# CZY-Code/PHNet

Hardware: AMD Instinct MI355X
Metric: clips/s (5x3x320x800) fwd+bwd (higher is better)
Workload: dtype f32 storage / accumulation, every product as an EXACT three-term bf16 split (6 bf16 MFMAs, f32-MFMA accuracy); 1 GPU; 5-frame clip 3x320x800, resnet34 + router + lane head, fwd+bwd+AdamW, 1 clip/GPU/step, random-init weights; parallelism=dp1, launch=hipGraph replay of the whole step

## Files before the change

### include/phnet_hip.h

```cpp
#ifndef PHNET_HIP_H
#define PHNET_HIP_H
#include <stdint.h>
#ifdef __cplusplus
extern "C" {
#endif

#define PHNET_OK 0
#define PHNET_ERR_ARG (-1)
#define PHNET_ERR_WORKSPACE (-2)
#define PHNET_ERR_LAUNCH (-3)
#define PHNET_ABI_VERSION 1

int phnet_abi_version(void);

int phnet_lane_nms(const float* rows, const float* scores, const int32_t* counts, int64_t frames,
                   int64_t k_max, int32_t n_offsets, float thresh, int64_t top_k,
                   int64_t* keep, int64_t* num_to_keep, int64_t* parent, void* stream);

int phnet_lane_decode(const float* lines, int64_t frames, int32_t N, int32_t n_offsets, float conf_thresh,
                      float nms_thresh, int64_t top_k, float img_w, uint8_t* keep_mask, int64_t* num,
                      int64_t* keep_c, int64_t* anchors, int64_t* anchors_sorted, float* kept_rows, void* stream);

int phnet_lane_points(const float* kept_rows, const int64_t* num, const float* prior_ys, int64_t F, int32_t L, int32_t S,
                      float* points, int32_t* count, int32_t* lanes_num, int32_t* slot, void* stream);
// ... 14 lines not shown
int phnet_lane_targets_aug(const float* points, const int32_t* counts, const int32_t* lanes_num, const double* offsets_ys, float* out,
                           int64_t F, int32_t Lin, int32_t P, int32_t R, int32_t S, double img_h, double img_w, double strip_size,
                           double crop, double src_w, double scale_x, double scale_y, int32_t flip, const int32_t* flip2,
                           const double* fwd, void* stream);
int phnet_lane_targets_clip(const float* points, const int32_t* counts, const int32_t* lanes_num, const double* offsets_ys, float* out,
                            int64_t F, int32_t Lin, int32_t P, int32_t R, int32_t S, double img_h, double img_w, double strip_size,
                            double crop, double src_w, double scale_x, double scale_y, int32_t flip, const int32_t* flip2,
                            const double* fwd, int32_t clip, int32_t* frag_count, void* stream);

int phnet_roi_pool_fwd(const float* fmap, const float* xs, const float* ys, float* out, float* out_cp,
                       int32_t B, int32_t N, int32_t P, int32_t h, int32_t w, int32_t C, void* stream);
int phnet_roi_pool_bwd(const float* dout, const float* fmap, const float* xs, const float* ys,
                       float* dmap, float* dxs,
                       int32_t B, int32_t N, int32_t P, int32_t h, int32_t w, int32_t C, void* stream);

int phnet_conv2d_fwd(const float* x, const float* w, const float* bias, float* y,
                     int32_t N, int32_t Hi, int32_t Wi, int32_t Ci, int32_t Co, int32_t R, int32_t S,
                     int32_t stride, int32_t pad, int32_t relu, void* workspace, uint64_t ws_bytes, void* stream);
uint64_t phnet_conv2d_stats_blocks(int64_t M, int32_t Co, int32_t K, uint64_t ws_bytes);
int phnet_conv2d_fwd_fused(const float* x, const float* w, const float* bias, const float* addend, float* y, float* stats,
                           int32_t N, int32_t Hi, int32_t Wi, int32_t Ci, int32_t Co, int32_t R, int32_t S,
                           int32_t stride, int32_t pad, int32_t relu, void* workspace, uint64_t ws_bytes, void* stream);
int phnet_conv2d_dgrad(const float* dy, const float* w, const float* addend, float* dx,
                       int32_t N, int32_t Hi, int32_t Wi, int32_t Ci, int32_t Co, int32_t R, int32_t S,
                       int32_t stride, int32_t pad, void* workspace, uint64_t ws_bytes, void* stream);
int phnet_conv3p_applies(int64_t M, int32_t Ca, int32_t Nn);
uint64_t phnet_conv3p_packed_bytes(int32_t Co, int32_t Ci);
int phnet_conv3p_pack(const float* w, void* packed, int32_t Co, int32_t Ci, int32_t dgrad, void* stream);
int phnet_conv3p_pack_jobs(const void* jobs, int32_t njobs, int64_t total, void* stream);
uint64_t phnet_conv3p_stats_blocks(int64_t M, int32_t Ca, int32_t Nn, uint64_t ws_bytes);
int phnet_conv3p_fwd(const float* x, const void* packed, const float* bias, const float* addend, float* y, float* stats,
                     int32_t N, int32_t H, int32_t W, int32_t Ca, int32_t Nn, int32_t relu,
                     void* workspace, uint64_t ws_bytes, void* stream);
int phnet_conv2d_plan(int64_t M, int32_t Co, int32_t K, uint64_t ws_bytes, int32_t* bm, int32_t* bn, int32_t* splits,
                      int32_t* k_tile);
int phnet_conv2d_kernel(int32_t dgrad, int32_t N, int32_t Hi, int32_t Wi, int32_t Ci, int32_t Co, int32_t R, int32_t S,
                        int32_t stride, int32_t pad, uint64_t ws_bytes, char* name, int32_t name_cap, int32_t* splits);
int phnet_conv2d_wgrad_kernel(int32_t N, int32_t Hi, int32_t Wi, int32_t Ci, int32_t Co, int32_t R, int32_t S, int32_t stride,
                              int32_t pad, int32_t has_dbias, uint64_t ws_bytes, char* name, int32_t name_cap, int32_t* splits);
int phnet_linear_bwd_kernel(int32_t M, int32_t K, int32_t N, int32_t has_relu_mask, char* name, int32_t name_cap);
int phnet_conv3p_kernel(int64_t M, int32_t Ca, int32_t Nn, uint64_t ws_bytes, char* name, int32_t name_cap, int32_t* splits);
uint64_t phnet_conv2d_wgrad_workspace(int32_t N, int32_t Hi, int32_t Wi, int32_t Ci, int32_t Co,
                                      int32_t R, int32_t S, int32_t stride, int32_t pad);
int phnet_conv2d_wgrad(const float* dy, const float* x, float* dw, float* dbias,
                       int32_t N, int32_t Hi, int32_t Wi, int32_t Ci, int32_t Co, int32_t R, int32_t S,
                       int32_t stride, int32_t pad, int32_t accumulate, void* workspace, uint64_t ws_bytes, void* stream);
int phnet_linear_bwd_fusable(int64_t M, int64_t K, int64_t N);
int phnet_linear_bwd(const float* dy, const float* x, const float* w, const float* relu_y, float* dx, float* dw, float* dbias,
                     int32_t M, int32_t K, int32_t N, int32_t accumulate, void* stream);
int phnet_nchw3_to_nhwc4(const float* x, float* y, int32_t N, int32_t H, int32_t W, void* stream);
int phnet_pad_channels(const float* src, float* dst, int64_t rows, int32_t cs, int32_t cd, void* stream);

uint64_t phnet_ipc_buffer_bytes(int32_t world, uint64_t max_bytes);
int phnet_ipc_alloc(uint64_t bytes, void** ptr);
int phnet_ipc_free(void* ptr);
int phnet_ipc_get_handle(void* ptr, void* handle64);
int phnet_ipc_open_handle(const void* handle64, void** ptr);
int phnet_ipc_close_handle(void* ptr);
int phnet_oneshot_allreduce(void* data, int32_t count, int32_t dtype, const void* peers, int32_t rank, int32_t world,
                            int32_t cap, void* ctrl, void* stream);

uint64_t phnet_channel_partials_size(int64_t M, int32_t C);
int phnet_bn_fwd_stats(const float* x, int64_t M, int32_t C, float eps, float momentum,
                       const float* gamma, const float* beta, float* running_mean, float* running_var,
                       float* save_mean, float* save_invstd, float* scale, float* shift,
                       float* partial, int32_t training, void* stream);
int phnet_bn_finalize_partials(const float* partial, int64_t nblk, int64_t M, int32_t C, float eps, float momentum,
                               const float* gamma, const float* beta, float* running_mean, float* running_var,
                               float* save_mean, float* save_invstd, float* scale, float* shift, void* stream);
int phnet_bn_apply(const float* x, const float* scale, const float* shift, const float* residual, float* y,
                   int64_t M, int32_t C, int32_t relu, void* stream);
int phnet_bn_bwd(const float* dy, const float* x, const float* y, const float* save_mean,
                 const float* save_invstd, const float* gamma, float* dx, float* dres,
                 float* dgamma, float* dbeta, float* partial, float* c1, float* c2,
                 int64_t M, int32_t C, int32_t relu, int32_t dres_accumulate, int32_t param_accumulate, void* stream);

int phnet_bn_bwd_reduce(const float* dy, const float* x, const float* y, const float* mean, const float* invstd,
                        float* sums, float* partial, float* c1_scratch, float* c2_scratch,
                        int64_t M, int32_t C, int32_t relu, void* stream);
int phnet_bn_bwd_apply(const float* dy, const float* x, const float* y, const float* mean, const float* invstd,
                       const float* gamma, const float* c1, const float* c2, float* dx, float* dres,
                       int64_t M, int32_t C, int32_t relu, int32_t dres_accumulate, void* stream);

int phnet_bn_local_sums(const float* x, int64_t M, int32_t C, float* partial, double* sums, void* stream);
int phnet_bn_partials_to_sums(const float* partial, int64_t nblk, int64_t M, int32_t C, double* sums, void* stream);
int phnet_bn_finalize_sums(const double* sums, int32_t C, float eps, float momentum, const float* gamma, const float* beta,
                           float* running_mean, float* running_var, float* save_mean, float* save_invstd,
                           float* scale, float* shift, void* stream);
int phnet_bn_bwd_apply_sums(const float* dy, const float* x, const float* y, const float* mean, const float* invstd,
                            const float* gamma, const float* sums, const double* count, float* c1, float* c2,
                            float* dx, float* dres, int64_t M, int32_t C, int32_t relu, int32_t dres_accumulate, void* stream);

int phnet_preprocess_u8(const uint8_t* frames, float* out, uint8_t* out_u8,
                        const int32_t* xi, const int16_t* xc, const int32_t* yi, const int16_t* yc,
                        int32_t T, int32_t H0, int32_t W0, int32_t crop_top, int32_t out_h, int32_t out_w, int32_t flip,
                        int32_t layout, const float* mean3_host, const float* std3_host, void* stream);
int phnet_preprocess_yuv(const uint8_t* frames, float* out, uint8_t* out_u8,
                         const int32_t* xi, const int16_t* xc, const int32_t* yi, const int16_t* yc,
                         int32_t T, int32_t H0, int32_t W0, int32_t crop_top, int32_t out_h, int32_t out_w, int32_t flip, int32_t layout,
                         int32_t format, int64_t frame_stride, int32_t pitch, int64_t chroma_offset,
                         const int32_t* csc_host, const float* mean3_host, const float* std3_host, void* stream);

int phnet_augment_u8(const uint8_t* frames, float* out, uint8_t* out_u8, const int32_t* flip2, const double* inv, const int32_t* table,
                     int32_t T, int32_t H, int32_t W, int32_t layout, const float* mean3_host, const float* std3_host, void* stream);

int phnet_augment_stencil_u8(const uint8_t* frames, float* out, uint8_t* out_u8, const int32_t* flip2, const double* inv,
                             const int32_t* table, const int32_t* stencil, uint8_t* staged, int32_t T, int32_t H, int32_t W, int32_t layout,
                             const float* mean3_host, const float* std3_host, void* stream);
// ... 197 lines not shown
```

### include/phnet_hip_tuning.h

```cpp
#ifndef PHNET_HIP_TUNING_H
#define PHNET_HIP_TUNING_H
#include <stdint.h>
#ifdef __cplusplus
extern "C" {
#endif

int phnet_tune_force_conv_tile(int32_t bm, int32_t bn, int32_t splits);
int phnet_tune_force_k_tile(int32_t k_tile);
int phnet_tune_wgrad(int32_t allow_bm128, int32_t target_blocks);
int phnet_tune_mma(int32_t mode);
int phnet_conv3p_tune(int32_t target_workgroups);
int phnet_tune_gate_wave(int32_t on);
int phnet_tune_dyn_mfma(int32_t on);
int phnet_tune_reset(void);
int phnet_tune_mma_get(void);

#ifdef __cplusplus
}
#endif
#endif
```

### phnet_amd/csrc/conv3p.hip

```cpp
#include <cstdio>
#include "igemm.h"
#include "tuning.h"

using namespace igemm;

namespace {

struct P3Shape {
    int N, H, W;
    int Ca, Nn;
    int splits, units_per_split;
};

constexpr int P3_BM = 128, P3_ROWS = P3_BM + 2, P3_THREADS = 256;
constexpr int P3_APITCH = 48;
constexpr int P3_ZROW = P3_ROWS;
constexpr int P3_APLANE = (P3_ROWS + 1) * P3_APITCH, P3_AIMG = 3 * P3_APLANE;
constexpr int P3_PFB = 3;
constexpr size_t P3_LDS = 2 * P3_AIMG + 3 * 512;

struct P3PackJob { const float* w; unsigned char* dst; int Co, Ci, dgrad, pad_; long first; };

__device__ __forceinline__ void conv3p_pack_item(const float* __restrict__ w, unsigned char* __restrict__ packed, int Co, int Ci,
                                                 int dgrad, long i)
// ... 331 lines not shown
{
    if (!w || !packed || Co < 16 || Ci < 16) return PHNET_ERR_ARG;
    const int Ca = dgrad ? Co : Ci, Nn = dgrad ? Ci : Co;
    if ((Ca % 16) || (Nn % 32)) return PHNET_ERR_ARG;
    const long total = (long)9 * (Ca / 16) * (Nn / 32) * 64;
    hipLaunchKernelGGL(conv3p_pack_kernel, dim3((unsigned)cdiv(total, 256)), dim3(256), 0, (hipStream_t)stream,
                       w, (unsigned char*)packed, Co, Ci, dgrad);
    return phnet_launch_status();
}

PHNET_API int phnet_conv3p_pack_jobs(const void* jobs, int32_t njobs, int64_t total, void* stream)
{
    if (!jobs || njobs < 1 || total < 1) return PHNET_ERR_ARG;
    hipLaunchKernelGGL(conv3p_pack_jobs_kernel, dim3((unsigned)cdiv((long)total, 256)), dim3(256), 0, (hipStream_t)stream,
                       (const P3PackJob*)jobs, njobs, (long)total);
    return phnet_launch_status();
}

PHNET_API uint64_t phnet_conv3p_stats_blocks(int64_t M, int32_t Ca, int32_t Nn, uint64_t ws_bytes)
{
    if (!p3_applies((long)M, Ca, Nn)) return 0;
    const P3Plan p = p3_plan((long)M, Ca, Nn, (size_t)ws_bytes);
    return (uint64_t)(p.splits > 1 ? cdiv((long)M * Nn / 4, 256 * P3_RCH) : cdiv((long)M, P3_BM) * (P3_BM / 64));
}

PHNET_API int phnet_conv3p_kernel(int64_t M, int32_t Ca, int32_t Nn, uint64_t ws_bytes, char* name, int32_t name_cap, int32_t* splits)
{
    if (!p3_applies((long)M, Ca, Nn) || !name || name_cap < 1 || !splits) return PHNET_ERR_ARG;
    const P3Plan p = p3_plan((long)M, Ca, Nn, (size_t)ws_bytes);
    *splits = p.splits;
    return p3_kernel_name(p, name, name_cap);
}

PHNET_API int phnet_conv3p_fwd(const float* x, const void* packed, const float* bias, const float* addend, float* y, float* stats,
                               int32_t N, int32_t H, int32_t W, int32_t Ca, int32_t Nn, int32_t relu,
                               void* workspace, uint64_t ws_bytes, void* stream)
{
    if (N < 0 || H < 1 || W < 2 || Ca < 16 || Nn < 64) return PHNET_ERR_ARG;
    if (N == 0) return PHNET_OK;
    const long M = (long)N * H * W;
    if (!x || !packed || !y || !p3_applies(M, Ca, Nn)) return PHNET_ERR_ARG;
    if (stats && (bias || addend || relu || (Nn & (Nn - 1)) || Nn > 1024)) return PHNET_ERR_ARG;
    const P3Plan p = p3_plan(M, Ca, Nn, workspace ? (size_t)ws_bytes : 0);
    P3Shape g{N, H, W, Ca, Nn, p.splits, p.units_per_split};
    float* dst = p.splits > 1 ? (float*)workspace : y;
    hipStream_t st = (hipStream_t)stream;
    if (p.fn == 2)
        hipLaunchKernelGGL(conv3p_kernel<2>, dim3((unsigned)p.tiles, 1, (unsigned)p.splits), dim3(P3_THREADS), P3_LDS, st,
                           x, (const unsigned char*)packed, bias, addend, dst, g, relu, p.splits > 1 ? (float*)nullptr : stats);
    else
        hipLaunchKernelGGL(conv3p_kernel<1>, dim3((unsigned)p.tiles, 1, (unsigned)p.splits), dim3(P3_THREADS), P3_LDS, st,
                           x, (const unsigned char*)packed, bias, addend, dst, g, relu, p.splits > 1 ? (float*)nullptr : stats);
    if (p.splits > 1) {
        const long total4 = M * Nn / 4;
        hipLaunchKernelGGL(conv3p_reduce_kernel, dim3((unsigned)cdiv(total4, stats ? 256 * P3_RCH : 256)), dim3(256), 0, st,
                           (const float*)workspace, y, bias, addend, total4, Nn, p.splits, relu, stats);
    }
    return phnet_launch_status();
}
```

### phnet_amd/csrc/norm.hip

```cpp
#include "common.h"

namespace {

typedef float f32x4 __attribute__((ext_vector_type(4)));
constexpr int NT = 256;

template <int MODE>
__global__ __launch_bounds__(NT) void channel_partials_kernel(
    const float* __restrict__ x, const float* __restrict__ dy, const float* __restrict__ y,
    const float* __restrict__ mean, const float* __restrict__ invstd,
    float* __restrict__ partial, long M, int C, long rows_per_block, int relu)
{
    extern __shared__ f32x4 red[];
    const int lanes_per_row = C >> 2;
    const int rows_at_once = NT / lanes_per_row;
    const int cl = threadIdx.x % lanes_per_row, rl = threadIdx.x / lanes_per_row;
    const long r0 = (long)blockIdx.x * rows_per_block;
    const long r1 = min(M, r0 + rows_per_block);
    f32x4 s0 = {0.f, 0.f, 0.f, 0.f}, s1 = {0.f, 0.f, 0.f, 0.f};
    f32x4 mu = {0.f, 0.f, 0.f, 0.f}, is = {0.f, 0.f, 0.f, 0.f};
    if (MODE == 1) {
        mu = *reinterpret_cast<const f32x4*>(mean + cl * 4);
        is = *reinterpret_cast<const f32x4*>(invstd + cl * 4);
    }
    for (long r = r0 + rl; r < r1; r += rows_at_once) {
        const size_t o = (size_t)r * C + cl * 4;
        const f32x4 xv = *reinterpret_cast<const f32x4*>(x + o);
        if (MODE == 0) {
            s0 += xv;
            s1 += xv * xv;
        } else {
            f32x4 g = *reinterpret_cast<const f32x4*>(dy + o);
            if (relu) {
                const f32x4 yv = *reinterpret_cast<const f32x4*>(y + o);
                g.x = yv.x > 0.f ? g.x : 0.f; g.y = yv.y > 0.f ? g.y : 0.f;
                g.z = yv.z > 0.f ? g.z : 0.f; g.w = yv.w > 0.f ? g.w : 0.f;
            }
            s0 += g;
            s1 += g * ((xv - mu) * is);
        }
    }
    red[threadIdx.x] = s0;
    red[NT + threadIdx.x] = s1;
    __syncthreads();
    if (rl == 0) {
        for (int k = 1; k < rows_at_once; ++k) {
            s0 += red[k * lanes_per_row + cl];
            s1 += red[NT + k * lanes_per_row + cl];
        }
        float* p = partial + (size_t)blockIdx.x * 2 * C;
        *reinterpret_cast<f32x4*>(p + cl * 4) = s0;
        *reinterpret_cast<f32x4*>(p + C + cl * 4) = s1;
    }
}

__device__ __forceinline__ double wave_sum_f64(double v) {
#pragma unroll
    for (int off = 32; off > 0; off >>= 1) v += __shfl_xor(v, off, 64);
    return v;
}

constexpr int FIN_CH = 8, FIN_NT = 1024, FIN_G = FIN_NT / FIN_CH;

__device__ __forceinline__ void finalize_column_sums(const float* __restrict__ partial, int nblk, int C, double* red, double& s0, double& s1)
{
    const int cl = threadIdx.x % FIN_CH, g = threadIdx.x / FIN_CH;
    const int c = blockIdx.x * FIN_CH + cl;
    double a = 0.0, b = 0.0;
    if (c < C) {
        constexpr int U = 8;
        for (int r = g; r < nblk; r += U * FIN_G) {
            float v[U], w[U];
#pragma unroll
            for (int u = 0; u < U; ++u) {
                const int rr = r + u * FIN_G;
                const size_t o = (size_t)(rr < nblk ? rr : g) * 2 * C + c;
                v[u] = partial[o];
                w[u] = partial[o + C];
            }
#pragma unroll
            for (int u = 0; u < U; ++u) {
                const bool in = r + u * FIN_G < nblk;
                a += in ? (double)v[u] : 0.0;
                b += in ? (double)w[u] : 0.0;
            }
// ... 329 lines not shown
}

PHNET_API int phnet_bn_apply(const float* x, const float* scale, const float* shift, const float* residual, float* y,
                             int64_t M, int32_t C, int32_t relu, void* stream)
{
    if (M < 1 || !channels_ok(C) || !x || !scale || !shift || !y) return PHNET_ERR_ARG;
    const long total4 = M * C / 4;
    hipLaunchKernelGGL(bn_apply_kernel, dim3((unsigned)ceil_div64(total4, NT)), dim3(NT), 0, (hipStream_t)stream,
                       x, scale, shift, residual, y, total4, C, relu);
    return phnet_launch_status();
}

PHNET_API int phnet_bn_bwd(const float* dy, const float* x, const float* y, const float* save_mean,
                           const float* save_invstd, const float* gamma, float* dx, float* dres,
                           float* dgamma, float* dbeta, float* partial, float* c1, float* c2,
                           int64_t M, int32_t C, int32_t relu, int32_t dres_accumulate, int32_t param_accumulate, void* stream)
{
    if (M < 1 || !channels_ok(C) || !dy || !x || !save_mean || !save_invstd || !gamma || !dx || !dgamma || !dbeta ||
        !partial || !c1 || !c2 || (relu && !y))
        return PHNET_ERR_ARG;
    hipStream_t st = (hipStream_t)stream;
    long rpb;
    const int nblk = (int)stat_blocks(M, &rpb);
    hipLaunchKernelGGL(channel_partials_kernel<1>, dim3(nblk), dim3(NT), 2 * NT * sizeof(f32x4), st,
                       x, dy, y, save_mean, save_invstd, partial, (long)M, C, rpb, relu);
    hipLaunchKernelGGL(bn_bwd_finalize_kernel, dim3((C + FIN_CH - 1) / FIN_CH), dim3(FIN_NT), 0, st, partial, nblk, (long)M, C,
                       dgamma, dbeta, c1, c2, param_accumulate);
    const long total4 = M * C / 4;
    hipLaunchKernelGGL(bn_bwd_apply_kernel, dim3((unsigned)ceil_div64(total4, NT)), dim3(NT), 0, st,
                       dy, x, y, save_mean, save_invstd, gamma, c1, c2, dx, dres, total4, C, relu, dres_accumulate);
    return phnet_launch_status();
}

PHNET_API int phnet_bn_bwd_reduce(const float* dy, const float* x, const float* y, const float* mean, const float* invstd,
                                  float* sums, float* partial, float* c1_scratch, float* c2_scratch,
                                  int64_t M, int32_t C, int32_t relu, void* stream)
{
    if (M < 1 || !channels_ok(C) || !dy || !x || !mean || !invstd || !sums || !partial || !c1_scratch || !c2_scratch || (relu && !y))
        return PHNET_ERR_ARG;
    hipStream_t st = (hipStream_t)stream;
    long rpb;
    const int nblk = (int)stat_blocks(M, &rpb);
    hipLaunchKernelGGL(channel_partials_kernel<1>, dim3(nblk), dim3(NT), 2 * NT * sizeof(f32x4), st,
                       x, dy, y, mean, invstd, partial, (long)M, C, rpb, relu);
    hipLaunchKernelGGL(bn_bwd_finalize_kernel, dim3((C + FIN_CH - 1) / FIN_CH), dim3(FIN_NT), 0, st, partial, nblk, (long)M, C,
                       sums, sums + C, c1_scratch, c2_scratch, 0);
    return phnet_launch_status();
}

PHNET_API int phnet_bn_bwd_apply(const float* dy, const float* x, const float* y, const float* mean, const float* invstd,
                                 const float* gamma, const float* c1, const float* c2, float* dx, float* dres,
                                 int64_t M, int32_t C, int32_t relu, int32_t dres_accumulate, void* stream)
{
    if (M < 1 || !channels_ok(C) || !dy || !x || !mean || !invstd || !gamma || !c1 || !c2 || !dx || (relu && !y))
        return PHNET_ERR_ARG;
    const long total4 = M * C / 4;
    hipLaunchKernelGGL(bn_bwd_apply_kernel, dim3((unsigned)ceil_div64(total4, NT)), dim3(NT), 0, (hipStream_t)stream,
                       dy, x, y, mean, invstd, gamma, c1, c2, dx, dres, total4, C, relu, dres_accumulate);
    return phnet_launch_status();
}

PHNET_API int phnet_bn_local_sums(const float* x, int64_t M, int32_t C, float* partial, double* sums, void* stream)
{
    if (M < 1 || !channels_ok(C) || !x || !partial || !sums) return PHNET_ERR_ARG;
    hipStream_t st = (hipStream_t)stream;
    long rpb;
// ... 106 lines not shown
```

### phnet_amd/csrc/tuning.h

```cpp
#pragma once

struct Tuning {
    int mma_mode = 3;
    int pf = 4;
    int buf_loads = 1;
    int uniform_tap = 1;
    int taps3 = 1;
    int deep_kt3 = 64;
    int force_bm = 0, force_bn = 0, force_splits = 0;
    int force_kt = 0;
    int wgrad_bm128 = 1;
    int wgrad_smallp = 1;
    int wgrad_bkw = 16;
    int wgrad3 = 1;
    int wgrad3_bkw = 16;
    int wgrad3s = 1;
    int wgrad1s = 1;
    int wgrad_target = 768;
    int wgrad3_target = 256;
    int smallp_max_tiles = 400;
    int p3_target = 512;
    int p3_wide = 1;
    int gate_wave = 1;
    int dyn_mfma = 1;
    int dyn_rows = 1;
};

Tuning& tuning();
```

### phnet_amd/csrc/tuning.hip

```cpp
#include "common.h"
#include "tuning.h"

Tuning& tuning() { static Tuning t; return t; }

PHNET_API int phnet_tune_reset(void) { tuning() = Tuning{}; return PHNET_OK; }
PHNET_API int phnet_tune_mma_get(void) { return tuning().mma_mode; }

PHNET_API int phnet_tune_force_conv_tile(int32_t bm, int32_t bn, int32_t splits)
{
    if (bm != 0 && !((bm == 64 || bm == 128) && (bn == 64 || bn == 128))) return PHNET_ERR_ARG;
    Tuning& t = tuning();
    t.force_bm = bm; t.force_bn = bn; t.force_splits = splits;
    return PHNET_OK;
}

PHNET_API int phnet_tune_force_k_tile(int32_t kt)
{
    Tuning& t = tuning();
    if (kt == -1 || kt == -2) { t.uniform_tap = kt == -2; return PHNET_OK; }
    if (kt == -5 || kt == -6) { t.taps3 = kt == -6; return PHNET_OK; }
    if (kt == -32 || kt == -64) { t.deep_kt3 = -kt; return PHNET_OK; }
    if (kt == -101 || kt == -102 || kt == -104) { t.pf = -kt - 100; return PHNET_OK; }
    if (kt == -200 || kt == -201) { t.buf_loads = -kt - 200; return PHNET_OK; }
    if (kt != 0 && kt != 16 && kt != 32 && kt != 64) return PHNET_ERR_ARG;
    t.force_kt = kt;
    return PHNET_OK;
}

PHNET_API int phnet_tune_wgrad(int32_t allow_bm128, int32_t target_blocks)
{
    if (target_blocks == 0 || target_blocks < -1024) return PHNET_ERR_ARG;
    Tuning& t = tuning();
    t.wgrad_bm128 = allow_bm128 & 1; t.wgrad_smallp = !(allow_bm128 & 2); t.wgrad_bkw = (allow_bm128 & 4) ? 32 : 16;
    t.wgrad3 = !(allow_bm128 & 8); t.wgrad3_bkw = (allow_bm128 & 16) ? 32 : 16;
    t.wgrad3s = !(allow_bm128 & 32); t.wgrad1s = !(allow_bm128 & 64);
    (target_blocks < 0 ? t.wgrad3_target : t.wgrad_target) = target_blocks < 0 ? -target_blocks : target_blocks;
    return PHNET_OK;
}

PHNET_API int phnet_tune_mma(int32_t mode)
{
    if (mode < 0 || mode > 3) return PHNET_ERR_ARG;
    tuning().mma_mode = mode;
    tuning().pf = mode == 3 ? 4 : 1;
    return PHNET_OK;
}

PHNET_API int phnet_conv3p_tune(int32_t target_workgroups)
{
    if (target_workgroups == -1 || target_workgroups == -2) { tuning().p3_wide = target_workgroups == -2; return PHNET_OK; }
    if (target_workgroups < 1) return PHNET_ERR_ARG;
    tuning().p3_target = target_workgroups;
    return PHNET_OK;
}

PHNET_API int phnet_tune_gate_wave(int32_t on) { tuning().gate_wave = on != 0; return PHNET_OK; }
PHNET_API int phnet_tune_dyn_mfma(int32_t on) { tuning().dyn_mfma = (on & 1) != 0; tuning().dyn_rows = !(on & 2); return PHNET_OK; }
```

### phnet_amd/hip_ops.py

```python
import ctypes
import os
from typing import Optional, Tuple

import torch

from ._lib import check, lib

_WS = {}

TIMER = None


def _kernel(query, *shape_args, has_splits=True):
    name, splits = ctypes.create_string_buffer(96), ctypes.c_int32(0)
    check(query(*shape_args, name, len(name), *([ctypes.byref(splits)] if has_splits else [])), "kernel query")
    return name.value.decode(), splits.value


def _timed_launch(sym_fn, flops, launch, shape=None, nbytes=None):
    if TIMER is None:
        return launch()
    sym, splits = sym_fn()
    e0, e1 = torch.cuda.Event(enable_timing=True), torch.cuda.Event(enable_timing=True)
    e0.record()
# ... 134 lines not shown

class Conv3pPackPlan:

    def __init__(self, weights, with_dgrad: bool = True):
        dev = weights[0].device
        self.ptrs = tuple(int(w.data_ptr()) for w in weights)
        sizes = [int(lib().phnet_conv3p_packed_bytes(w.shape[0], w.shape[3])) for w in weights]
        kinds = (False, True) if with_dgrad else (False,)
        self.buf = torch.empty(sum(sizes) * len(kinds), dtype=torch.uint8, device=dev)
        self.images, rows, off, first = [], [], 0, 0
        for w, nbytes in zip(weights, sizes):
            _req(w, name="w")
            co, _, _, ci = w.shape
            per = {}
            for dg in kinds:
                ca, nn = (co, ci) if dg else (ci, co)
                assert ca % 16 == 0 and nn % 32 == 0, w.shape
                img = self.buf[off:off + nbytes]
                rows.append([int(w.data_ptr()), int(img.data_ptr()), co | (ci << 32), int(dg), first])
                first += 9 * (ca // 16) * (nn // 32) * 64
                off += nbytes
                per[dg] = img
            self.images.append(per)
        self.total = first
        self.jobs = torch.tensor(rows, dtype=torch.int64).to(dev)

    def matches(self, weights) -> bool:
        return self.ptrs == tuple(int(w.data_ptr()) for w in weights)

    def refresh(self):
        check(lib().phnet_conv3p_pack_jobs(_ptr(self.jobs), self.jobs.shape[0], self.total, _stream()), "phnet_conv3p_pack_jobs")


def conv3p(x: torch.Tensor, packed: torch.Tensor, nn: int, dgrad: bool = False, bias=None, addend=None, relu: bool = False,
           stats: bool = False):
    _req(x, name="x")
    n, h, w_, ca = x.shape
    out = torch.empty((n, h, w_, nn), dtype=torch.float32, device=x.device)
    m = n * h * w_
    need = 8 * m * nn * 4 if m * nn < (1 << 23) else 0
    ws = workspace(need, x.device) if need else None
    part, nblk = None, 0
    if stats:
        nblk = int(lib().phnet_conv3p_stats_blocks(m, ca, nn, need))
        part = workspace(nblk * 2 * nn * 4, x.device, 1)
    if addend is not None:
        _req(addend, name="addend")
        assert addend.shape == out.shape
    _timed_launch(lambda: _kernel(lib().phnet_conv3p_kernel, m, ca, nn, need),
                  2.0 * m * nn * 9 * ca,
                  lambda: check(lib().phnet_conv3p_fwd(_ptr(x), _ptr(packed), _ptr(bias), _ptr(addend), _ptr(out), _ptr(part), n, h, w_, ca, nn,
                                                       int(relu), _ptr(ws), need, _stream()), "phnet_conv3p_fwd"),
                  shape=("dgrad" if dgrad else "fwd", m, nn, 9 * ca, 3),
                  nbytes=4.0 * m * (ca + nn) + 6.0 * 9 * ca * nn + (4.0 * m * nn if addend is not None else 0.0))
    return (out, (part, nblk)) if stats else out


def conv2d_dgrad(dy, w, in_hw: Tuple[int, int], stride: int, pad: int, addend: Optional[torch.Tensor] = None,
                 out: Optional[torch.Tensor] = None):
    _req(dy, name="dy"); _req(w, name="w")
    n = dy.shape[0]
    co, r, s, ci = w.shape
    hi, wi = in_hw
    dx = torch.empty((n, hi, wi, ci), dtype=torch.float32, device=dy.device) if out is None else _req(out, name="out")
    assert dx.shape == (n, hi, wi, ci)
    need = 8 * n * hi * wi * ci * 4 if n * hi * wi * ci < (1 << 23) else 0
    ws = workspace(need, dy.device) if need else None
    m, k = n * hi * wi, r * s * co
    _timed_launch(lambda: _kernel(lib().phnet_conv2d_kernel, 1, n, hi, wi, ci, co, r, s, stride, pad, need), 2.0 * dy.shape[0] * dy.shape[1] * dy.shape[2] * co * r * s * ci,
                  lambda: check(lib().phnet_conv2d_dgrad(_ptr(dy), _ptr(w), _ptr(addend), _ptr(dx), n, hi, wi, ci, co, r, s, stride,
                                                         pad, _ptr(ws), need, _stream()), "phnet_conv2d_dgrad"),
                  shape=("dgrad", m, ci, k, r), nbytes=4.0 * (dy.numel() + m * ci + co * r * s * ci))
    return dx


CONV3P = os.environ.get("PHNET_CONV3P", "1") != "0"


def conv2d_wgrad(dy, x, w_shape, stride: int, pad: int, dw: Optional[torch.Tensor] = None, accumulate: bool = False,
                 dbias: Optional[torch.Tensor] = None):
    _req(dy, name="dy"); _req(x, name="x")
# ... 66 lines not shown

def _partials(m, c, device, slot=1):
    nfloats = lib().phnet_channel_partials_size(m, c)
    return workspace(nfloats * 4, device, slot)


def bn_fwd(x, gamma, beta, running_mean, running_var, training: bool, eps: float, momentum: float,
           residual=None, relu: bool = True, partials=None):
    _req(x, name="x")
    c = x.shape[-1]
    m = x.numel() // c
    dev = x.device
    scale = torch.empty(c, dtype=torch.float32, device=dev)
    shift = torch.empty(c, dtype=torch.float32, device=dev)
    sm = torch.empty(c, dtype=torch.float32, device=dev) if training else None
    si = torch.empty(c, dtype=torch.float32, device=dev) if training else None
    if training and partials is not None:
        check(lib().phnet_bn_finalize_partials(_ptr(partials[0]), int(partials[1]), m, c, eps, momentum, _ptr(gamma), _ptr(beta),
                                               _ptr(running_mean), _ptr(running_var), _ptr(sm), _ptr(si), _ptr(scale), _ptr(shift),
                                               _stream()), "phnet_bn_finalize_partials")
    else:
        part = _partials(m, c, dev) if training else None
        check(lib().phnet_bn_fwd_stats(_ptr(x), m, c, eps, momentum, _ptr(gamma), _ptr(beta), _ptr(running_mean),
                                       _ptr(running_var), _ptr(sm), _ptr(si), _ptr(scale), _ptr(shift), _ptr(part),
                                       int(training), _stream()), "phnet_bn_fwd_stats")
    y = torch.empty_like(x)
    check(lib().phnet_bn_apply(_ptr(x), _ptr(scale), _ptr(shift), _ptr(residual), _ptr(y), m, c, int(relu), _stream()),
          "phnet_bn_apply")
    return y, sm, si


def bn_bwd(dy, x, y, save_mean, save_invstd, gamma, relu: bool, dres: Optional[torch.Tensor] = None,
           dres_accumulate: bool = False, dgamma: Optional[torch.Tensor] = None, dbeta: Optional[torch.Tensor] = None,
           param_accumulate: bool = False):
    _req(dy, name="dy")
    c = x.shape[-1]
    m = x.numel() // c
    dev = x.device
    dx = torch.empty_like(x)
    dgamma = torch.empty(c, dtype=torch.float32, device=dev) if dgamma is None else dgamma
    dbeta = torch.empty(c, dtype=torch.float32, device=dev) if dbeta is None else dbeta
    c12 = torch.empty(2, c, dtype=torch.float32, device=dev)
    part = _partials(m, c, dev)
    check(lib().phnet_bn_bwd(_ptr(dy), _ptr(x), _ptr(y), _ptr(save_mean), _ptr(save_invstd), _ptr(gamma), _ptr(dx),
                             _ptr(dres), _ptr(dgamma), _ptr(dbeta), _ptr(part), _ptr(c12[0]), _ptr(c12[1]),
                             m, c, int(relu), int(dres_accumulate), int(param_accumulate), _stream()), "phnet_bn_bwd")
    return dx, dgamma, dbeta


def bn_fwd_sync(x, gamma, beta, running_mean, running_var, eps: float, momentum: float, residual=None, relu: bool = True,
                group=None, partials=None):
    from . import parallel
    _req(x, name="x")
    c = x.shape[-1]
    m = x.numel() // c
    dev = x.device
    stats = torch.empty(4, c, dtype=torch.float32, device=dev)
    sums = torch.empty(2 * c + 1, dtype=torch.float64, device=dev)
    if partials is not None and partials[0] is not None:
        check(lib().phnet_bn_partials_to_sums(_ptr(partials[0]), int(partials[1]), m, c, _ptr(sums), _stream()), "phnet_bn_partials_to_sums")
    else:
        part = _partials(m, c, dev)
        check(lib().phnet_bn_local_sums(_ptr(x), m, c, _ptr(part), _ptr(sums), _stream()), "phnet_bn_local_sums")
    parallel.allreduce_sum_(sums, group)
    check(lib().phnet_bn_finalize_sums(_ptr(sums), c, eps, momentum, _ptr(gamma), _ptr(beta), _ptr(running_mean), _ptr(running_var),
                                       _ptr(stats[0]), _ptr(stats[1]), _ptr(stats[2]), _ptr(stats[3]), _stream()), "phnet_bn_finalize_sums")
    y = torch.empty_like(x)
    check(lib().phnet_bn_apply(_ptr(x), _ptr(stats[2]), _ptr(stats[3]), _ptr(residual), _ptr(y), m, c, int(relu), _stream()),
          "phnet_bn_apply")
    return y, stats[0], stats[1], sums[2 * c:]


def bn_bwd_sync(dy, x, y, mean, invstd, gamma, relu: bool, count, dres: Optional[torch.Tensor] = None, group=None,
                dres_accumulate: bool = False, dgamma: Optional[torch.Tensor] = None, dbeta: Optional[torch.Tensor] = None,
                param_accumulate: bool = False):
    from . import parallel
# ... 1089 lines not shown
    if pred.dim() < 2 or pred.shape != gt.shape or pred.device != gt.device:
        raise ValueError(f"mask_metric_counts: pred {tuple(pred.shape)} and gt {tuple(gt.shape)} must be u8 [.., H, W] of one shape on one device")
    lead, (h, w) = tuple(pred.shape[:-2]), pred.shape[-2:]
    radius = int(radius)
    if not (1 <= h <= MASK_METRICS_MAX_SIZE and 1 <= w <= MASK_METRICS_MAX_SIZE):
        raise ValueError(f"mask_metric_counts: height and width must be in 1..{MASK_METRICS_MAX_SIZE}, got {h} x {w}")
    if not 0 <= radius <= MASK_METRICS_MAX_RADIUS:
        raise ValueError(f"mask_metric_counts: radius must be in 0..{MASK_METRICS_MAX_RADIUS}, got {radius}")
    n = 1
    for d in lead:
        n *= int(d)
    if out is None:
        out = torch.empty(lead + (7,), dtype=torch.int64, device=pred.device)
    else:
        _req(out, torch.int64, "out")
        if tuple(out.shape) != lead + (7,) or out.device != pred.device:
            raise ValueError(f"mask_metric_counts: out must be int64 {lead + (7,)} on {pred.device}, got {tuple(out.shape)}")
    if n == 0:
        return out
    nbytes = lib().phnet_mask_metrics_workspace(n, h, w, radius)
    ws = workspace(nbytes, pred.device)
    check(lib().phnet_mask_metrics(_ptr(pred), _ptr(gt), n, h, w, radius, _ptr(ws), ws.numel(), _ptr(out), _stream()), "phnet_mask_metrics")
    return out


def tune_k_tile(code: int) -> None:
    check(lib().phnet_tune_force_k_tile(code), "phnet_tune_force_k_tile")


def tune_wgrad(flags: int = 1, target: int = 768) -> None:
    check(lib().phnet_tune_wgrad(flags, target), "phnet_tune_wgrad")


def tune_reset() -> None:
    check(lib().phnet_tune_reset(), "phnet_tune_reset")


def mma_mode() -> int:
    return int(lib().phnet_tune_mma_get())


def set_mma_mode(mode: str) -> None:
    check(lib().phnet_tune_mma({"f32": 0, "split_bf16": 1, "split3_bf16": 2, "bf16x3": 3}[mode]), "phnet_tune_mma")
```

### phnet_amd/trunk.py

```python
from typing import Callable, List, Optional

import torch
import torch.nn as nn

from . import hip_ops as K
from .arena import direct_grad

STAGE_DONE_HOOK: Optional[Callable[[str], None]] = None
PARTS = ("head", "neck", "layer4", "layer3", "layer2", "layer1", "stem")


def ohwi(w: torch.Tensor) -> torch.Tensor:
    return w.detach().permute(0, 2, 3, 1).contiguous()


def oihw_grad(dw_ohwi: torch.Tensor) -> torch.Tensor:
    return dw_ohwi.permute(0, 3, 1, 2)


def _sync_bn(bn) -> bool:
    from . import parallel
    return isinstance(bn, nn.SyncBatchNorm) and parallel.active(getattr(bn, "process_group", None))


# ... 200 lines not shown
    for i in range(3):
        m = neck.fpn_convs[i].conv
        conv_wgrad_into(m.weight, douts[i], ctx.lats[i], ctx.out_w[i].shape, 1, 1, bias=m.bias)
        if ctx.out_packs[i] is not None and K.conv3p_applies(douts[i].shape[0] * douts[i].shape[1] * douts[i].shape[2],
                                                             ctx.out_w[i].shape[0], ctx.out_w[i].shape[3]):
            dl.append(K.conv3p(douts[i], ctx.out_packs[i][True], ctx.out_w[i].shape[3], dgrad=True))
        else:
            dl.append(K.conv2d_dgrad(douts[i], ctx.out_w[i], tuple(ctx.lats[i].shape[1:3]), 1, 1))
    for i in (1, 2):
        K.upsample_add_bwd_(dl[i - 1], dl[i])
    dstage = []
    for i in range(3):
        m = neck.lateral_convs[i].conv
        conv_wgrad_into(m.weight, dl[i], ctx.feats[i], ctx.lat_w[i].shape, 1, 0, bias=m.bias)
        dstage.append(K.conv2d_dgrad(dl[i], ctx.lat_w[i], tuple(ctx.feats[i].shape[1:3]), 1, 0))
    done("neck")
    tape = ctx.tape
    pos = len(tape)

    def bn_back(rec, dy, dres=None, dres_acc=False):
        dgd, dbd = direct_grad(rec.bn.weight), direct_grad(rec.bn.bias)
        direct = dgd is not None and dbd is not None
        kw = dict(dgamma=dgd, dbeta=dbd, param_accumulate=True) if direct else {}
        if rec.sync_count is not None:
            dx, dg, db = K.bn_bwd_sync(dy, rec.c, rec.y, rec.sm, rec.si, rec.bn.weight.detach(), rec.relu, rec.sync_count, dres,
                                       getattr(rec.bn, "process_group", None), dres_accumulate=dres_acc, **kw)
        else:
            dx, dg, db = K.bn_bwd(dy, rec.c, rec.y, rec.sm, rec.si, rec.bn.weight.detach(), rec.relu, dres, dres_acc, **kw)
        if not direct:
            put(rec.bn.weight, dg)
            put(rec.bn.bias, db)
        return dx

    def conv_back(rec, dc, need_dx=True, addend=None):
        if rec.conv is model.conv1:
            dw = K.conv2d_wgrad(dc, rec.x_in, rec.w.shape, rec.stride, rec.pad)
            dw = oihw_grad(K.pad_channels(dw.view(-1, 4), 3).view(dw.shape[0], 7, 7, 3))
            d = direct_grad(rec.conv.weight)
            if d is not None:
                d.add_(dw)
            else:
                put(rec.conv.weight, dw)
        else:
            conv_wgrad_into(rec.conv.weight, dc, rec.x_in, rec.w.shape, rec.stride, rec.pad)
        if not need_dx:
            return None
        if rec.packed is not None:
            return K.conv3p(dc, rec.packed[True], rec.w.shape[3], dgrad=True, addend=addend)
        return K.conv2d_dgrad(dc, rec.w, tuple(rec.x_in.shape[1:3]), rec.stride, rec.pad, addend)

    dy = None
    stage_names = ("layer4", "layer3", "layer2", "layer1")
    for si, name in enumerate(stage_names):
        extra = dstage[2 - si] if si < 3 else None
        if dy is None:
            dy = extra
        elif extra is not None:
            dy = dy + extra
        for blk in reversed(list(getattr(model, name))):
            has_ds = blk.downsample is not None
            rec2 = tape[pos - 1]
            recd = tape[pos - 2] if has_ds else None
            rec1 = tape[pos - 3] if has_ds else tape[pos - 2]
            pos -= 3 if has_ds else 2
            dres = torch.empty_like(rec2.c)
            dc2 = bn_back(rec2, dy, dres)
            dh = conv_back(rec2, dc2)
            dc1 = bn_back(rec1, dh)
            if has_ds:
                dcd = bn_back(recd, dres)
                dxd = conv_back(recd, dcd)
                dy = conv_back(rec1, dc1, addend=dxd)
            else:
                dy = conv_back(rec1, dc1, addend=dres)
        done(name)
    rec = tape[0]
    dpool = K.maxpool_bwd(dy, ctx.argmax, ctx.stem_shape)
    dc = bn_back(rec, dpool)
    conv_back(rec, dc, need_dx=False)
    done("stem")
    ctx.tape = ctx.feats = ctx.lats = None
    return grads


class EncoderFunction(torch.autograd.Function):

    @staticmethod
    def forward(ctx, enc, training: bool, frames: torch.Tensor, *params):
        outs, tape = encoder_fwd_schedule(enc, training, frames)
        if training:
            ctx.tape = tape
        return outs

    @staticmethod
    def backward(ctx, d3, d4, d5):
        grads = encoder_bwd_schedule(ctx.tape, d3, d4, d5, STAGE_DONE_HOOK)
        ctx.tape = None
        return (None, None, None, *grads)


def encoder_forward(enc, frames: torch.Tensor):
    params = [p for p in enc.parameters()]
    training = enc.training and torch.is_grad_enabled()
    if training and getattr(enc, "staged", False):
        return encoder_forward_staged(enc, frames)
    if enc.training and not training:
        return EncoderFunction.apply(enc, True, frames, *[p.detach() for p in params])
# ... 22 lines not shown
```

Before: 67.87 clips/s.

## Fuse conv3p dgrad split-K reduction into the following BN backward partials pass

After: 68.24 clips/s (median of 6 runs). About the same (+0.6%).

```diff
diff --git a/include/phnet_hip.h b/include/phnet_hip.h
--- a/include/phnet_hip.h
+++ b/include/phnet_hip.h
@@ -70,6 +70,9 @@
 int phnet_conv3p_fwd(const float* x, const void* packed, const float* bias, const float* addend, float* y, float* stats,
                      int32_t N, int32_t H, int32_t W, int32_t Ca, int32_t Nn, int32_t relu,
                      void* workspace, uint64_t ws_bytes, void* stream);
+int phnet_conv3p_dgrad_slabs(const float* x, const void* packed, const float* addend, float* y,
+                             int32_t N, int32_t H, int32_t W, int32_t Ca, int32_t Nn,
+                             void* workspace, uint64_t ws_bytes, int32_t* splits, void* stream);
 int phnet_conv2d_plan(int64_t M, int32_t Co, int32_t K, uint64_t ws_bytes, int32_t* bm, int32_t* bn, int32_t* splits,
                       int32_t* k_tile);
 int phnet_conv2d_kernel(int32_t dgrad, int32_t N, int32_t Hi, int32_t Wi, int32_t Ci, int32_t Co, int32_t R, int32_t S,
@@ -112,6 +115,10 @@
                  const float* save_invstd, const float* gamma, float* dx, float* dres,
                  float* dgamma, float* dbeta, float* partial, float* c1, float* c2,
                  int64_t M, int32_t C, int32_t relu, int32_t dres_accumulate, int32_t param_accumulate, void* stream);
+int phnet_bn_bwd_slabs(const float* slabs, int32_t splits, const float* addend, float* dy, const float* x, const float* y,
+                       const float* save_mean, const float* save_invstd, const float* gamma, float* dx, float* dres,
+                       float* dgamma, float* dbeta, float* partial, float* c1, float* c2,
+                       int64_t M, int32_t C, int32_t relu, int32_t dres_accumulate, int32_t param_accumulate, void* stream);
 
 int phnet_bn_bwd_reduce(const float* dy, const float* x, const float* y, const float* mean, const float* invstd,
                         float* sums, float* partial, float* c1_scratch, float* c2_scratch,
diff --git a/include/phnet_hip_tuning.h b/include/phnet_hip_tuning.h
--- a/include/phnet_hip_tuning.h
+++ b/include/phnet_hip_tuning.h
@@ -10,6 +10,8 @@
 int phnet_tune_wgrad(int32_t allow_bm128, int32_t target_blocks);
 int phnet_tune_mma(int32_t mode);
 int phnet_conv3p_tune(int32_t target_workgroups);
+int phnet_tune_bn_tail(int32_t on);
+int phnet_tune_bn_tail_get(void);
 int phnet_tune_gate_wave(int32_t on);
 int phnet_tune_dyn_mfma(int32_t on);
 int phnet_tune_reset(void);
diff --git a/phnet_amd/csrc/conv3p.hip b/phnet_amd/csrc/conv3p.hip
--- a/phnet_amd/csrc/conv3p.hip
+++ b/phnet_amd/csrc/conv3p.hip
@@ -387,29 +387,53 @@
     return p3_kernel_name(p, name, name_cap);
 }
 
-PHNET_API int phnet_conv3p_fwd(const float* x, const void* packed, const float* bias, const float* addend, float* y, float* stats,
-                               int32_t N, int32_t H, int32_t W, int32_t Ca, int32_t Nn, int32_t relu,
-                               void* workspace, uint64_t ws_bytes, void* stream)
-{
-    if (N < 0 || H < 1 || W < 2 || Ca < 16 || Nn < 64) return PHNET_ERR_ARG;
-    if (N == 0) return PHNET_OK;
+namespace {
+
+int p3_launch(const float* x, const void* packed, const float* bias, const float* addend, float* y, float* stats,
+              int N, int H, int W, int Ca, int Nn, int relu, void* workspace, size_t ws_bytes, bool defer, hipStream_t st)
+{
     const long M = (long)N * H * W;
-    if (!x || !packed || !y || !p3_applies(M, Ca, Nn)) return PHNET_ERR_ARG;
-    if (stats && (bias || addend || relu || (Nn & (Nn - 1)) || Nn > 1024)) return PHNET_ERR_ARG;
-    const P3Plan p = p3_plan(M, Ca, Nn, workspace ? (size_t)ws_bytes : 0);
+    const P3Plan p = p3_plan(M, Ca, Nn, workspace ? ws_bytes : 0);
     P3Shape g{N, H, W, Ca, Nn, p.splits, p.units_per_split};
     float* dst = p.splits > 1 ? (float*)workspace : y;
-    hipStream_t st = (hipStream_t)stream;
     if (p.fn == 2)
         hipLaunchKernelGGL(conv3p_kernel<2>, dim3((unsigned)p.tiles, 1, (unsigned)p.splits), dim3(P3_THREADS), P3_LDS, st,
                            x, (const unsigned char*)packed, bias, addend, dst, g, relu, p.splits > 1 ? (float*)nullptr : stats);
     else
         hipLaunchKernelGGL(conv3p_kernel<1>, dim3((unsigned)p.tiles, 1, (unsigned)p.splits), dim3(P3_THREADS), P3_LDS, st,
                            x, (const unsigned char*)packed, bias, addend, dst, g, relu, p.splits > 1 ? (float*)nullptr : stats);
-    if (p.splits > 1) {
+    if (p.splits > 1 && !defer) {
         const long total4 = M * Nn / 4;
         hipLaunchKernelGGL(conv3p_reduce_kernel, dim3((unsigned)cdiv(total4, stats ? 256 * P3_RCH : 256)), dim3(256), 0, st,
                            (const float*)workspace, y, bias, addend, total4, Nn, p.splits, relu, stats);
     }
+    return p.splits;
+}
+
+}
+
+PHNET_API int phnet_conv3p_fwd(const float* x, const void* packed, const float* bias, const float* addend, float* y, float* stats,
+                               int32_t N, int32_t H, int32_t W, int32_t Ca, int32_t Nn, int32_t relu,
+                               void* workspace, uint64_t ws_bytes, void* stream)
+{
+    if (N < 0 || H < 1 || W < 2 || Ca < 16 || Nn < 64) return PHNET_ERR_ARG;
+    if (N == 0) return PHNET_OK;
+    const long M = (long)N * H * W;
+    if (!x || !packed || !y || !p3_applies(M, Ca, Nn)) return PHNET_ERR_ARG;
+    if (stats && (bias || addend || relu || (Nn & (Nn - 1)) || Nn > 1024)) return PHNET_ERR_ARG;
+    p3_launch(x, packed, bias, addend, y, stats, N, H, W, Ca, Nn, relu, workspace, (size_t)ws_bytes, false, (hipStream_t)stream);
     return phnet_launch_status();
 }
+
+PHNET_API int phnet_conv3p_dgrad_slabs(const float* x, const void* packed, const float* addend, float* y,
+                                       int32_t N, int32_t H, int32_t W, int32_t Ca, int32_t Nn,
+                                       void* workspace, uint64_t ws_bytes, int32_t* splits, void* stream)
+{
+    if (N < 1 || H < 1 || W < 2 || Ca < 16 || Nn < 64 || !splits) return PHNET_ERR_ARG;
+    const long M = (long)N * H * W;
+    if (!x || !packed || !y || !p3_applies(M, Ca, Nn)) return PHNET_ERR_ARG;
+    const bool defer = tuning().bn_tail != 0;
+    const int s = p3_launch(x, packed, nullptr, addend, y, nullptr, N, H, W, Ca, Nn, 0, workspace, (size_t)ws_bytes, defer, (hipStream_t)stream);
+    *splits = defer ? s : 1;
+    return phnet_launch_status();
+}
diff --git a/phnet_amd/csrc/norm.hip b/phnet_amd/csrc/norm.hip
--- a/phnet_amd/csrc/norm.hip
+++ b/phnet_amd/csrc/norm.hip
@@ -51,6 +51,73 @@
         float* p = partial + (size_t)blockIdx.x * 2 * C;
         *reinterpret_cast<f32x4*>(p + cl * 4) = s0;
         *reinterpret_cast<f32x4*>(p + C + cl * 4) = s1;
+    }
+}
+
+constexpr int SLAB_U = 4;
+
+template <int ZMAX>
+__global__ __launch_bounds__(NT) void channel_partials_slabs_kernel(
+    const float* __restrict__ x, const float* __restrict__ part, int splits, const float* __restrict__ addend,
+    float* __restrict__ dy, const float* __restrict__ y, const float* __restrict__ mean, const float* __restrict__ invstd,
+    float* __restrict__ partial, long M, int C, long rows_per_block, int relu)
+{
+    extern __shared__ f32x4 red[];
+    const int lanes_per_row = C >> 2;
+    const int rows_at_once = NT / lanes_per_row;
+    const int cl = threadIdx.x % lanes_per_row, rl = threadIdx.x / lanes_per_row;
+    const long r0 = (long)blockIdx.x * rows_per_block;
+    const long r1 = min(M, r0 + rows_per_block);
+    const long total4 = M * C / 4;
+    f32x4 s0 = {0.f, 0.f, 0.f, 0.f}, s1 = {0.f, 0.f, 0.f, 0.f};
+    const f32x4 mu = *reinterpret_cast<const f32x4*>(mean + cl * 4);
+    const f32x4 is = *reinterpret_cast<const f32x4*>(invstd + cl * 4);
+    const float* ym = relu ? y : x;
+    const float* am = addend ? addend : x;
+    for (long r = r0 + rl; r < r1; r += (long)SLAB_U * rows_at_once) {
+        size_t o[SLAB_U];
+        f32x4 xv[SLAB_U], yv[SLAB_U], av[SLAB_U], v[SLAB_U][ZMAX];
+#pragma unroll
+        for (int u = 0; u < SLAB_U; ++u) {
+            const long rr = r + (long)u * rows_at_once;
+            o[u] = (size_t)(rr < r1 ? rr : r) * C + cl * 4;
+            xv[u] = *reinterpret_cast<const f32x4*>(x + o[u]);
+            yv[u] = *reinterpret_cast<const f32x4*>(ym + o[u]);
+            av[u] = *reinterpret_cast<const f32x4*>(am + o[u]);
+            const f32x4* p = reinterpret_cast<const f32x4*>(part + o[u]);
+#pragma unroll
+            for (int z = 0; z < ZMAX; ++z) v[u][z] = p[(long)min(z, splits - 1) * total4];
+        }
+#pragma unroll
+        for (int u = 0; u < SLAB_U; ++u) {
+            if (r + (long)u * rows_at_once >= r1) break;
+            f32x4 s = v[u][0];
+#pragma unroll
+            for (int z = 1; z < ZMAX; ++z)
+                if (z < splits) s += v[u][z];
+            for (int z = ZMAX; z < splits; ++z) s += reinterpret_cast<const f32x4*>(part + o[u])[(long)z * total4];
+            if (addend) s += av[u];
+            *reinterpret_cast<f32x4*>(dy + o[u]) = s;
+            f32x4 g = s;
+            if (relu) {
+                g.x = yv[u].x > 0.f ? g.x : 0.f; g.y = yv[u].y > 0.f ? g.y : 0.f;
+                g.z = yv[u].z > 0.f ? g.z : 0.f; g.w = yv[u].w > 0.f ? g.w : 0.f;
+            }
+            s0 += g;
+            s1 += g * ((xv[u] - mu) * is);
+        }
+    }
+    red[threadIdx.x] = s0;
+    red[NT + threadIdx.x] = s1;
+    __syncthreads();
+    if (rl == 0) {
+        for (int k = 1; k < rows_at_once; ++k) {
+            s0 += red[k * lanes_per_row + cl];
+            s1 += red[NT + k * lanes_per_row + cl];
+        }
+        float* q = partial + (size_t)blockIdx.x * 2 * C;
+        *reinterpret_cast<f32x4*>(q + cl * 4) = s0;
+        *reinterpret_cast<f32x4*>(q + C + cl * 4) = s1;
     }
 }
 
@@ -446,6 +513,31 @@
     return phnet_launch_status();
 }
 
+PHNET_API int phnet_bn_bwd_slabs(const float* slabs, int32_t splits, const float* addend, float* dy, const float* x, const float* y,
+                                 const float* save_mean, const float* save_invstd, const float* gamma, float* dx, float* dres,
+                                 float* dgamma, float* dbeta, float* partial, float* c1, float* c2,
+                                 int64_t M, int32_t C, int32_t relu, int32_t dres_accumulate, int32_t param_accumulate, void* stream)
+{
+    if (M < 1 || !channels_ok(C) || splits < 1 || !slabs || !dy || !x || !save_mean || !save_invstd || !gamma || !dx || !dgamma ||
+        !dbeta || !partial || !c1 || !c2 || (relu && !y))
+        return PHNET_ERR_ARG;
+    hipStream_t st = (hipStream_t)stream;
+    long rpb;
+    const int nblk = (int)stat_blocks(M, &rpb);
+    if (splits <= 4)
+        hipLaunchKernelGGL(channel_partials_slabs_kernel<4>, dim3(nblk), dim3(NT), 2 * NT * sizeof(f32x4), st,
+                           x, slabs, splits, addend, dy, y, save_mean, save_invstd, partial, (long)M, C, rpb, relu);
+    else
+        hipLaunchKernelGGL(channel_partials_slabs_kernel<8>, dim3(nblk), dim3(NT), 2 * NT * sizeof(f32x4), st,
+                           x, slabs, splits, addend, dy, y, save_mean, save_invstd, partial, (long)M, C, rpb, relu);
+    hipLaunchKernelGGL(bn_bwd_finalize_kernel, dim3((C + FIN_CH - 1) / FIN_CH), dim3(FIN_NT), 0, st, partial, nblk, (long)M, C,
+                       dgamma, dbeta, c1, c2, param_accumulate);
+    const long total4 = M * C / 4;
+    hipLaunchKernelGGL(bn_bwd_apply_kernel, dim3((unsigned)ceil_div64(total4, NT)), dim3(NT), 0, st,
+                       (const float*)dy, x, y, save_mean, save_invstd, gamma, c1, c2, dx, dres, total4, C, relu, dres_accumulate);
+    return phnet_launch_status();
+}
+
 PHNET_API int phnet_bn_bwd_reduce(const float* dy, const float* x, const float* y, const float* mean, const float* invstd,
                                   float* sums, float* partial, float* c1_scratch, float* c2_scratch,
                                   int64_t M, int32_t C, int32_t relu, void* stream)
diff --git a/phnet_amd/csrc/tuning.h b/phnet_amd/csrc/tuning.h
--- a/phnet_amd/csrc/tuning.h
+++ b/phnet_amd/csrc/tuning.h
@@ -21,6 +21,7 @@
     int smallp_max_tiles = 400;
     int p3_target = 512;
     int p3_wide = 1;
+    int bn_tail = 1;
     int gate_wave = 1;
     int dyn_mfma = 1;
     int dyn_rows = 1;
diff --git a/phnet_amd/csrc/tuning.hip b/phnet_amd/csrc/tuning.hip
--- a/phnet_amd/csrc/tuning.hip
+++ b/phnet_amd/csrc/tuning.hip
@@ -54,5 +54,7 @@
     return PHNET_OK;
 }
 
+PHNET_API int phnet_tune_bn_tail(int32_t on) { tuning().bn_tail = on != 0; return PHNET_OK; }
+PHNET_API int phnet_tune_bn_tail_get(void) { return tuning().bn_tail; }
 PHNET_API int phnet_tune_gate_wave(int32_t on) { tuning().gate_wave = on != 0; return PHNET_OK; }
 PHNET_API int phnet_tune_dyn_mfma(int32_t on) { tuning().dyn_mfma = (on & 1) != 0; tuning().dyn_rows = !(on & 2); return PHNET_OK; }
diff --git a/phnet_amd/hip_ops.py b/phnet_amd/hip_ops.py
--- a/phnet_amd/hip_ops.py
+++ b/phnet_amd/hip_ops.py
@@ -190,11 +190,19 @@
         check(lib().phnet_conv3p_pack_jobs(_ptr(self.jobs), self.jobs.shape[0], self.total, _stream()), "phnet_conv3p_pack_jobs")
 
 
+class SlabGradient:
+    __slots__ = ("out", "slabs", "splits", "addend")
+
+    def __init__(self, out, slabs, splits, addend):
+        self.out, self.slabs, self.splits, self.addend = out, slabs, splits, addend
+
+
 def conv3p(x: torch.Tensor, packed: torch.Tensor, nn: int, dgrad: bool = False, bias=None, addend=None, relu: bool = False,
-           stats: bool = False):
+           stats: bool = False, defer: bool = False, out: Optional[torch.Tensor] = None):
     _req(x, name="x")
     n, h, w_, ca = x.shape
-    out = torch.empty((n, h, w_, nn), dtype=torch.float32, device=x.device)
+    out = torch.empty((n, h, w_, nn), dtype=torch.float32, device=x.device) if out is None else _req(out, name="out")
+    assert out.shape == (n, h, w_, nn)
     m = n * h * w_
     need = 8 * m * nn * 4 if m * nn < (1 << 23) else 0
     ws = workspace(need, x.device) if need else None
@@ -205,6 +213,17 @@
     if addend is not None:
         _req(addend, name="addend")
         assert addend.shape == out.shape
+    if defer:
+        assert dgrad and bias is None and not relu and not stats
+        splits = ctypes.c_int32(0)
+        _timed_launch(lambda: _kernel(lib().phnet_conv3p_kernel, m, ca, nn, need),
+                      2.0 * m * nn * 9 * ca,
+                      lambda: check(lib().phnet_conv3p_dgrad_slabs(_ptr(x), _ptr(packed), _ptr(addend), _ptr(out), n, h, w_, ca, nn,
+                                                                   _ptr(ws), need, ctypes.byref(splits), _stream()),
+                                    "phnet_conv3p_dgrad_slabs"),
+                      shape=("dgrad", m, nn, 9 * ca, 3),
+                      nbytes=4.0 * m * (ca + nn) + 6.0 * 9 * ca * nn + (4.0 * m * nn if addend is not None else 0.0))
+        return out if splits.value == 1 else SlabGradient(out, ws, splits.value, addend)
     _timed_launch(lambda: _kernel(lib().phnet_conv3p_kernel, m, ca, nn, need),
                   2.0 * m * nn * 9 * ca,
                   lambda: check(lib().phnet_conv3p_fwd(_ptr(x), _ptr(packed), _ptr(bias), _ptr(addend), _ptr(out), _ptr(part), n, h, w_, ca, nn,
@@ -337,16 +356,24 @@
 
 def bn_bwd(dy, x, y, save_mean, save_invstd, gamma, relu: bool, dres: Optional[torch.Tensor] = None,
            dres_accumulate: bool = False, dgamma: Optional[torch.Tensor] = None, dbeta: Optional[torch.Tensor] = None,
-           param_accumulate: bool = False):
-    _req(dy, name="dy")
+           param_accumulate: bool = False, dx: Optional[torch.Tensor] = None):
+    slabs = dy if isinstance(dy, SlabGradient) else None
+    dy = _req(dy.out if slabs is not None else dy, name="dy")
     c = x.shape[-1]
     m = x.numel() // c
     dev = x.device
-    dx = torch.empty_like(x)
+    dx = torch.empty_like(x) if dx is None else _req(dx, name="dx")
     dgamma = torch.empty(c, dtype=torch.float32, device=dev) if dgamma is None else dgamma
     dbeta = torch.empty(c, dtype=torch.float32, device=dev) if dbeta is None else dbeta
     c12 = torch.empty(2, c, dtype=torch.float32, device=dev)
     part = _partials(m, c, dev)
+    if slabs is not None:
+        assert dy.shape == x.shape
+        check(lib().phnet_bn_bwd_slabs(_ptr(slabs.slabs), slabs.splits, _ptr(slabs.addend), _ptr(dy), _ptr(x), _ptr(y), _ptr(save_mean),
+                                       _ptr(save_invstd), _ptr(gamma), _ptr(dx), _ptr(dres), _ptr(dgamma), _ptr(dbeta), _ptr(part),
+                                       _ptr(c12[0]), _ptr(c12[1]), m, c, int(relu), int(dres_accumulate), int(param_accumulate),
+                                       _stream()), "phnet_bn_bwd_slabs")
+        return dx, dgamma, dbeta
     check(lib().phnet_bn_bwd(_ptr(dy), _ptr(x), _ptr(y), _ptr(save_mean), _ptr(save_invstd), _ptr(gamma), _ptr(dx),
                              _ptr(dres), _ptr(dgamma), _ptr(dbeta), _ptr(part), _ptr(c12[0]), _ptr(c12[1]),
                              m, c, int(relu), int(dres_accumulate), int(param_accumulate), _stream()), "phnet_bn_bwd")
@@ -1502,6 +1529,10 @@
     check(lib().phnet_tune_wgrad(flags, target), "phnet_tune_wgrad")
 
 
+def tune_bn_tail(on: bool) -> None:
+    check(lib().phnet_tune_bn_tail(int(on)), "phnet_tune_bn_tail")
+
+
 def tune_reset() -> None:
     check(lib().phnet_tune_reset(), "phnet_tune_reset")
 
diff --git a/phnet_amd/trunk.py b/phnet_amd/trunk.py
--- a/phnet_amd/trunk.py
+++ b/phnet_amd/trunk.py
@@ -256,7 +256,7 @@
             put(rec.bn.bias, db)
         return dx
 
-    def conv_back(rec, dc, need_dx=True, addend=None):
+    def conv_back(rec, dc, need_dx=True, addend=None, consumer=None):
         if rec.conv is model.conv1:
             dw = K.conv2d_wgrad(dc, rec.x_in, rec.w.shape, rec.stride, rec.pad)
             dw = oihw_grad(K.pad_channels(dw.view(-1, 4), 3).view(dw.shape[0], 7, 7, 3))
@@ -270,7 +270,8 @@
         if not need_dx:
             return None
         if rec.packed is not None:
-            return K.conv3p(dc, rec.packed[True], rec.w.shape[3], dgrad=True, addend=addend)
+            defer = consumer is not None and consumer.sync_count is None
+            return K.conv3p(dc, rec.packed[True], rec.w.shape[3], dgrad=True, addend=addend, defer=defer)
         return K.conv2d_dgrad(dc, rec.w, tuple(rec.x_in.shape[1:3]), rec.stride, rec.pad, addend)
 
     dy = None
@@ -281,7 +282,9 @@
             dy = extra
         elif extra is not None:
             dy = dy + extra
-        for blk in reversed(list(getattr(model, name))):
+        blocks = list(getattr(model, name))
+        for bi in range(len(blocks) - 1, -1, -1):
+            blk = blocks[bi]
             has_ds = blk.downsample is not None
             rec2 = tape[pos - 1]
             recd = tape[pos - 2] if has_ds else None
@@ -289,14 +292,14 @@
             pos -= 3 if has_ds else 2
             dres = torch.empty_like(rec2.c)
             dc2 = bn_back(rec2, dy, dres)
-            dh = conv_back(rec2, dc2)
+            dh = conv_back(rec2, dc2, consumer=rec1)
             dc1 = bn_back(rec1, dh)
             if has_ds:
                 dcd = bn_back(recd, dres)
                 dxd = conv_back(recd, dcd)
                 dy = conv_back(rec1, dc1, addend=dxd)
             else:
-                dy = conv_back(rec1, dc1, addend=dres)
+                dy = conv_back(rec1, dc1, addend=dres, consumer=tape[pos - 1] if bi > 0 else None)
         done(name)
     rec = tape[0]
     dpool = K.maxpool_bwd(dy, ctx.argmax, ctx.stem_shape)
```
